# JOP-Lee/READ

Measured on AMD Instinct MI355X. Metric: rendered frames/sec @1216x352, 30M pts, higher is better.
Workload: dtype f32 (matrix-core products from two f16 pieces per operand, three piece pairs, fp32 accumulation)

## Files before the change

include/read_hip.h:

```cpp
#ifndef READ_HIP_H
#define READ_HIP_H

#include <stddef.h>
#include <stdint.h>

#ifdef __cplusplus
extern "C" {
#endif

#define READ_OK        0
#define READ_EINVAL  (-22)
#define READ_ENOMEM  (-12)
#define READ_EHIP     (-5)

#define READ_MAX_LEVELS      5
#define READ_DESC_CHANNELS   8

const char *read_last_error(void);
int read_abi_version(void);
int read_device_arch(char *name, int len);

int read_tuning_set(const char *key, int value);
int read_tuning_get(const char *key, int *value);
const char *read_tuning_key(int i);
// ... 190 lines not shown
    const float *wpacked_sc;
    int pre_bilinear;
    const void *wpacked_w4h;
    const void *wpacked_d3h;
    const void *wpacked_t3h;
} read_conv_desc;

size_t read_conv_packed_floats(int Cin, int Cout, int ksize);
size_t read_conv_param_floats(int Cout);
int read_conv_pack_weights_host(int Cin, int Cout, int ksize, int kc, const float *wf,
                                const float *wm, float *wpacked_host);
size_t read_conv_wino_floats(int Cin, int Cout);
int read_conv_pack_wino_host(int Cin, int Cout, const float *wf, const float *wm, float *wpacked_wino_host);
int read_conv_pack_w16_host(int Cin, int Cout, const float *wf, const float *wm, float *wpacked_w16_host);
size_t read_conv_w4_floats(int Cin, int Cout);
int read_conv_pack_w4_host(int Cin, int Cout, const float *wf, const float *wm, float *wpacked_w4_host);
size_t read_conv_w4h_floats(int Cin, int Cout);
int read_conv_pack_w4h_host(int Cin, int Cout, const float *wf, const float *wm, void *wpacked_w4h_host);
size_t read_conv_d3h_floats(int Cin, int Cout);
int read_conv_pack_d3h_host(int Cin, int Cout, const float *wf, const float *wm, void *wpacked_d3h_host);
size_t read_conv_dkh_floats(int Cin, int Cout, int ksize);
int read_conv_pack_dkh_host(int Cin, int Cout, int ksize, const float *wf, const float *wm, void *wpacked_host);
size_t read_conv_t3h_floats(int Cin, int Cout);
int read_conv_pack_t3h_host(int Cin, int Cout, const float *wf, const float *wm, void *wpacked_t3h_host);
size_t read_conv_sc_floats(int Cin, int Cout);
int read_conv_pack_sc_host(int Cin, int Cout, const float *wf, const float *wm, float *wpacked_sc_host);
int read_conv_pack_params_host(int Cout, const float *bf, const float *bm, const float *gamma,
                               const float *beta, const float *mean, const float *var, float eps,
                               float *params_host);
int read_gated_conv_forward(const read_conv_desc *desc, void *stream);
size_t read_conv_f4x1_floats(int Cin, int Cout);
int read_conv_pack_f4x1_host(int Cin, int Cout, const float *wf, const float *wm, void *wpacked_f4x1_host);
int read_gated_conv_forward_f4x1(const read_conv_desc *desc, const void *wpacked_f4x1, void *stream);
int read_conv_unpack_weights_host(int Cin, int Cout, int ksize, int kc, const float *wpacked_host, float *wf, float *wm);
int read_conv_kernel_family(const read_conv_desc *desc);
int read_conv_config_count(void);
const char *read_conv_config_name(int config);

int read_bilinear_up4(const float *in, int inH, int inW, int C, float *out, void *stream);

enum { READ_PACK_PARAMS = 0, READ_PACK_DIRECT = 1, READ_PACK_WINO = 2, READ_PACK_W4 = 3 };
typedef struct read_pack_job {
    int kind, mode;
    int Cin, Cout, ksize, kc;
    int Cp, first_block, nblocks;
    float eps;
    const float *wf, *wm;
    const float *bf, *bm, *gamma, *beta, *mean, *var;
    float *out;
    long long total;
} read_pack_job;
int read_conv_pack_job_prepare(read_pack_job *job);
int read_conv_pack_job(read_pack_job *job_host, void *stream);
int read_conv_pack_batch(const read_pack_job *jobs_dev, int njobs, int total_blocks, void *stream);
int read_conv_pack_params_device(int Cout, const float *bf, const float *bm, const float *gamma, const float *beta,
                                 const float *mean, const float *var, float eps, float *params, void *stream);
int read_conv_pack_weights_device(int Cin, int Cout, int ksize, int kc, const float *wf, const float *wm, float *wpacked,
                                  void *stream);
int read_conv_pack_wino_device(int Cin, int Cout, const float *wf, const float *wm, float *wpacked_wino, void *stream);
int read_conv_pack_w4_device(int Cin, int Cout, const float *wf, const float *wm, float *wpacked_w4, void *stream);
size_t read_conv_dgrad_packed_floats(int Cin, int Cout, int ksize);
size_t read_conv_dgrad_wino_floats(int Cin, int Cout);
size_t read_conv_dgrad_w4_floats(int Cin, int Cout);
int read_conv_pack_dgrad_device(int Cin, int Cout, int ksize, int kc, const float *wf, const float *wm, float *wpacked,
                                void *stream);
int read_conv_pack_dgrad_wino_device(int Cin, int Cout, const float *wf, const float *wm, float *wpacked_wino, void *stream);
// ... 68 lines not shown
```

read_amd/_lib.py:

```python
import ctypes as C
import os

_HERE = os.path.dirname(os.path.abspath(__file__))
LIB_PATH = os.path.join(_HERE, "libreadhip_debug.so" if os.environ.get("READ_HIP_DEBUG") else "libreadhip.so")
if os.environ.get("READ_HIP_VARIANT"):
    LIB_PATH = os.path.join(_HERE, "libreadhip_v_%s.so" % os.environ["READ_HIP_VARIANT"])

READ_MAX_LEVELS = 5
READ_CONV_MAX_SRC = 4
DESC_CHANNELS = 8


class ReadHipError(RuntimeError):
    pass


class ConvSrc(C.Structure):
    _fields_ = [("data", C.c_void_p), ("C", C.c_int), ("srcH", C.c_int), ("srcW", C.c_int), ("shift", C.c_int)]


class ConvDesc(C.Structure):
    _fields_ = [
        ("n_src", C.c_int), ("src", ConvSrc * READ_CONV_MAX_SRC), ("mul", C.c_void_p),
        ("inH", C.c_int), ("inW", C.c_int), ("Cout", C.c_int), ("ksize", C.c_int), ("stride", C.c_int),
# ... 117 lines not shown
    "read_rows_to_texture": (_i, [_vp, _i64, _i, _vp, _vp]),
    "read_gather_forward": (_i, [_vp, _i64, _i, _i, _pp, C.POINTER(_i64), _pp, _i, _vp]),
    "read_gather_forward_ss": (_i, [_vp, _i64, _i, _i, _i, _pp, C.POINTER(_i), C.POINTER(_i), _i, _pp, _i, _vp]),
    "read_gather_forward_tables": (_i, [C.POINTER(GatherTable), _i, _i, _i, _pp, C.POINTER(_i64), _pp, _vp]),
    "read_gather_backward": (_i, [_vp, _i64, _i, _i, _pp, C.POINTER(_i64), _pp, _vp]),
    "read_stitch_gather_forward": (_i, [C.POINTER(StitchPart), _i, _i, _i, C.POINTER(_i64), _pp, _pp, _pp, _pp, _vp]),
    "read_bilinear_down": (_i, [_vp, _i64, _i, _i, _i, _vp, _vp]),
    "read_bilinear_down_backward": (_i, [_vp, _i64, _i, _i, _i, _vp, _vp]),
    "read_conv_packed_floats": (_sz, [_i, _i, _i]),
    "read_conv_param_floats": (_sz, [_i]),
    "read_conv_pack_weights_host": (_i, [_i, _i, _i, _i, _vp, _vp, _vp]),
    "read_conv_pack_params_host": (_i, [_i, _vp, _vp, _vp, _vp, _vp, _vp, _f, _vp]),
    "read_conv_wino_floats": (_sz, [_i, _i]),
    "read_conv_pack_wino_host": (_i, [_i, _i, _vp, _vp, _vp]),
    "read_conv_pack_w16_host": (_i, [_i, _i, _vp, _vp, _vp]),
    "read_conv_w4_floats": (_sz, [_i, _i]),
    "read_conv_pack_w4_host": (_i, [_i, _i, _vp, _vp, _vp]),
    "read_conv_w4h_floats": (_sz, [_i, _i]),
    "read_conv_pack_w4h_host": (_i, [_i, _i, _vp, _vp, _vp]),
    "read_conv_d3h_floats": (_sz, [_i, _i]),
    "read_conv_pack_d3h_host": (_i, [_i, _i, _vp, _vp, _vp]),
    "read_conv_t3h_floats": (_sz, [_i, _i]),
    "read_conv_pack_t3h_host": (_i, [_i, _i, _vp, _vp, _vp]),
    "read_conv_dkh_floats": (_sz, [_i, _i, _i]),
    "read_conv_pack_dkh_host": (_i, [_i, _i, _i, _vp, _vp, _vp]),
    "read_gated_conv_forward": (_i, [C.POINTER(ConvDesc), _vp]),
    "read_conv_f4x1_floats": (_sz, [_i, _i]),
    "read_conv_unpack_weights_host": (_i, [_i, _i, _i, _i, _vp, _vp, _vp]),
    "read_unet_f4x1_floats": (_sz, []),
    "read_unet_f4x1_layer": (_i, [_i, C.POINTER(_sz), C.POINTER(_sz), C.POINTER(_i), C.POINTER(_i)]),
    "read_unet_set_f4x1": (_i, [_vp, _vp]),
    "read_conv_pack_f4x1_host": (_i, [_i, _i, _vp, _vp, _vp]),
    "read_gated_conv_forward_f4x1": (_i, [C.POINTER(ConvDesc), _vp, _vp]),
    "read_conv_kernel_family": (_i, [_vp]),
    "read_conv_sc_floats": (_sz, [_i, _i]),
    "read_conv_pack_sc_host": (_i, [_i, _i, _vp, _vp, _vp]),
    "read_conv_pack_job_prepare": (_i, [C.POINTER(PackJob)]),
    "read_conv_pack_job": (_i, [C.POINTER(PackJob), _vp]),
    "read_conv_pack_batch": (_i, [_vp, _i, _i, _vp]),
    "read_conv_config_count": (_i, []),
    "read_conv_config_name": (C.c_char_p, [_i]),
    "read_bilinear_up4": (_i, [_vp, _i, _i, _i, _vp, _vp]),
    "read_conv_pack_params_device": (_i, [_i, _vp, _vp, _vp, _vp, _vp, _vp, _f, _vp, _vp]),
    "read_conv_pack_weights_device": (_i, [_i, _i, _i, _i, _vp, _vp, _vp, _vp]),
    "read_conv_pack_wino_device": (_i, [_i, _i, _vp, _vp, _vp, _vp]),
    "read_conv_dgrad_wino_floats": (_sz, [_i, _i]),
    "read_conv_pack_dgrad_wino_device": (_i, [_i, _i, _vp, _vp, _vp, _vp]),
    "read_conv_pack_w4_device": (_i, [_i, _i, _vp, _vp, _vp, _vp]),
    "read_conv_dgrad_w4_floats": (_sz, [_i, _i]),
    "read_conv_pack_dgrad_w4_device": (_i, [_i, _i, _vp, _vp, _vp, _vp]),
    "read_conv_dgrad_packed_floats": (_sz, [_i, _i, _i]),
    "read_conv_pack_dgrad_device": (_i, [_i, _i, _i, _i, _vp, _vp, _vp, _vp]),
    "read_gate_forward": (_i, [_vp, _i64, _i, _vp, _i, _vp, _vp, _i, _i, _i, _vp]),
    "read_gate_backward": (_i, [_vp, _vp, _i64, _i, _vp, _i, _vp, _vp, _i, _i, _i, _vp]),
    "read_bn_param_grads": (_i, [_i, _vp, _vp, _vp, _f, _vp, _vp, _vp, _vp, _vp]),
    "read_bn_train_forward": (_i, [_vp, _i64, _i, _i, _i, _i, _i, _vp, _vp, _f, _f, _vp, _vp, _vp, _vp, _vp, _vp]),
    "read_gate_backward_bn": (_i, [_vp, _vp, _i64, _i, _vp, _i, _vp, _vp, _i, _i, _i, _i, _vp, _vp, _f, _vp, _vp]),
    "read_bn_param_grads_groups": (_i, [_i, _i, _vp, _vp, _f, _vp, _vp, _vp, _vp, _vp]),
    "read_conv_dgrad_generic_floats": (_sz, [_i, _i, _i]),
    "read_conv_dgrad_generic": (_i, [_vp, _i, _i, _i, _i, _i, _i, _vp, _vp, _vp, _i, _i, _vp, _vp]),
    "read_conv_wgrad_scratch_floats": (_sz, [_i, _i, _i, _i]),
    "read_conv_wgrad": (_i, [_vp, _i, _i, _i, _vp, _i, _i, _i, _vp, _vp, _i, _vp, _sz, _vp]),
    "read_conv_wgrad_family": (_i, [_i, _i, _i, _i, _i]),
    "read_bilinear_up4_blocks": (_i, [_vp, _i, _i, _i, _vp, _i, _i, _vp]),
    "read_bilinear_up4_backward": (_i, [_vp, _i, _i, _i, _vp, _i, _i, _vp]),
    "read_huber_loss": (_i, [_vp, _vp, _i64, _f, _vp, _vp, _vp]),
# ... 95 lines not shown
```

read_amd/csrc/conv.hip:

```cpp
#include <limits.h>

#include "common.h"
#include "internal.h"

using namespace readhip;

typedef float floatx16 __attribute__((ext_vector_type(16)));

namespace {

constexpr long long OOB_LIMIT = 0x7ffffff0ll;

struct SrcDev {
    const float *p;
    int C, H, W;
    int sl, sr;
};

struct ConvKArgs {
    SrcDev src[READ_CONV_MAX_SRC];
    const float *mul;
    const float *wp;
    const float *wp_wino;
    const float *wp_w16;
// ... 2179 lines not shown
                    const auto sw = __builtin_amdgcn_permlane32_swap(u0[k], u1[k], false, false);
                    u0[k] = sw[0];
                    u1[k] = sw[1];
                }
                Yf[py][px] = __builtin_bit_cast(f32x4, u0);
                Ym[py][px] = __builtin_bit_cast(f32x4, u1);
            }
#pragma unroll
        for (int py = 0; py < 2; ++py)
#pragma unroll
            for (int px = 0; px < 4; ++px) {
                f32x4 f = __builtin_elementwise_fma(Yf[py][px], isf, bf);
                const f32x4 mm = __builtin_elementwise_fma(Ym[py][px], ism, bml);
                if (a.elu) {
                    const f32x4 fe = f * LOG2E;
                    f32x4 e;
#pragma unroll
                    for (int k = 0; k < 4; ++k) e[k] = __builtin_amdgcn_exp2f(fe[k]);
                    e = e + f32x4{-1.0f, -1.0f, -1.0f, -1.0f};
#pragma unroll
                    for (int k = 0; k < 4; ++k) f[k] = f[k] > 0.0f ? f[k] : e[k];
                }
                f32x4 sg_, t;
#pragma unroll
                for (int k = 0; k < 4; ++k) t[k] = __builtin_amdgcn_exp2f(mm[k]);
                t = t + f32x4{1.0f, 1.0f, 1.0f, 1.0f};
#pragma unroll
                for (int k = 0; k < 4; ++k) sg_[k] = __builtin_amdgcn_rcpf(t[k]);
                const f32x4 v = (f * sg_) * sc + sh + rv[py][px];
                __builtin_amdgcn_raw_buffer_store_b128(__builtin_bit_cast(u32x4, v), out_rsrc, ovoff[py][px], 0, 0);
            }
        step_tile(by, bx);
        __builtin_amdgcn_s_setprio(0);
    }
}

struct D3hGeom {
    static constexpr int IH = 10, IW = 34, NPIX = IH * IW;
    static constexpr int XBUF = NPIX * 32;
    static constexpr int NE = NPIX * 8, NI = (NE + 511) / 512;
};

template <bool MUL>
__global__ __launch_bounds__(512, 1) void gated_conv_d3h_kernel(const ConvKArgs a)
{
    using DG = D3hGeom;
    __shared__ __attribute__((aligned(16))) unsigned lds[2 * DG::XBUF];
    __shared__ __attribute__((aligned(16))) float epar[6][32];
    const int tid = threadIdx.x, lane = tid & 63;
    const int wv = __builtin_amdgcn_readfirstlane(tid >> 6), rh = wv & 1, pq = wv >> 1;
    const SrcDev s = a.src[0];
    const int groups = a.CoutPad >> 5, G = gridDim.x;
    const int g = blockIdx.x % groups;
    const int n = a.nchunks;
    constexpr unsigned OOR = 0x80000000u;

    int by = (blockIdx.x / groups) / a.tiles_x, bx = (blockIdx.x / groups) % a.tiles_x;
    int pby = by, pbx = bx, pu = blockIdx.x, pchunk = 0;
    auto step_tile = [&](int &ty_, int &tx_) {
        ty_ += a.wino_dby;
        tx_ += a.wino_dbx;
        if (tx_ >= a.tiles_x) {
            tx_ -= a.tiles_x;
            ++ty_;
        }
    };
// ... 1119 lines not shown
    CFGW(1, 1, 32, 2, 1, 1, 2),
    CFGW(1, 1, 32, 1, 1, 1, 4),
    CFGW(3, 1, 8, 2, 1, 2, 2),
    {"k3s1c16_p1q1_wino", 3, 1, 16, 1, 1, 4, 1, 1, 2, gated_conv_wino_kernel<false, false>, gated_conv_wino_kernel<false, true>, 0, 0, 1},
    CFG(4, 2, 16, 1, 1, 1, 1, 1),
    CFG(4, 2, 16, 1, 1, 4, 1, 1),
    CFG(4, 2, 16, 1, 2, 2, 2, 1),
};
constexpr int N_CONFIGS = sizeof(g_configs) / sizeof(g_configs[0]);

int find_config(int ks, int s, int kc, int P, int QG, int WM, int WN, int PF, int NB)
{
    for (int i = 0; i < N_CONFIGS; ++i) {
        const ConvConfig &c = g_configs[i];
        if (c.KS == ks && c.S == s && c.KC == kc && c.P == P && c.QG == QG && c.WM == WM && c.WN == WN && c.PF == PF &&
            c.NB == NB)
            return i;
    }
    return -1;
}

enum ConvForce {
    CFG_AUTO = -1,
    CFG_PX = -2,
    CFG_W16 = -3,
    CFG_W4 = -5,
    CFG_SC = -6,
    CFG_W4H = -7,
    CFG_D3H = -8,
    CFG_D3H_S2 = -9,
    CFG_PXH = -10,
    CFG_T3H = -11,
    CFG_F4X1 = -12,
};

int g_prefer_wave = 1;
int g_wino_wgs = 2;
int g_conv_px = 1;
int g_kc32 = 1;
int g_use_wino = 1 << 30;
int g_w4_grid = 0;
int g_w4 = 32;
int g_w4h = 32;
int g_f4x1 = 32;
int g_d3h = 0;
int g_d3h_fam = 32;
int g_d3h_s2 = 32;
int g_pxh = 16;
int g_t3h = 8;
int g_sc = 8;
int g_w16 = 0;
int g_stagger_ticks = 0;

int find_wave_config(int ks, int s, int kc, int P, int QG)
{
    int best = -1;
    for (int i = 0; i < N_CONFIGS; ++i) {
        const ConvConfig &c = g_configs[i];
        if (c.wave && c.KS == ks && c.S == s && c.KC == kc && c.P == P && c.QG == QG) best = i;
    }
    return best;
}

int first_fit(int ks, int s, int kc, int groups, bool tiled_only = false, bool with_mul = false)
{
    for (int i = 0; i < N_CONFIGS; ++i) {
// ... 538 lines not shown
{
    g_trace = (unsigned long long *)buf;
    g_trace_records = buf ? bytes / 64 : 0;
}


static int conv_uses_wino(const read_conv_desc *d)
{
    return d->config < 0 && g_use_wino && !d->pre && d->ksize == 3 && d->stride == 1 && d->n_src == 1 &&
           d->src[0].shift == 0 && d->src[0].C % 16 == 0 && d->wpacked_wino && d->src[0].C <= g_use_wino;
}

static int conv_uses_w4(const read_conv_desc *d)
{
    const bool shape = !d->pre && (!d->linear || !d->residual) && d->ksize == 3 && d->stride == 1 && d->n_src == 1 && d->src[0].shift == 0 &&
                       d->src[0].C % 16 == 0 && d->src[0].C >= 32 && (d->Cout % 32 == 0 || (d->linear && d->Cout % 8 == 0)) && !d->fill_pad && d->wpacked_w4 &&
                       d->out_cstride % 4 == 0 &&
                       (long long)d->src[0].srcH * d->src[0].srcW * d->src[0].C * 4 < (1ll << 31) &&
                       (long long)d->inH * d->inW * d->out_cstride * 4 < (1ll << 31);
    return shape && (d->config == CFG_W4 || (d->config == CFG_AUTO && g_w4 > 0 && d->src[0].C >= g_w4));
}

static int conv_w4_shape(const read_conv_desc *d, const void *operand, bool with_threshold = false)
{
    read_conv_desc t = *d;
    if (!with_threshold) t.config = CFG_W4;
    t.wpacked_w4 = reinterpret_cast<const float *>(operand);
    return conv_uses_w4(&t);
}

static int conv_uses_w4h(const read_conv_desc *d)
{
    if (!d->wpacked_w4h || d->linear || d->mul || d->src[0].C % 32 != 0 || d->Cout % 32 != 0) return 0;
    const bool forced = d->config == CFG_W4H || d->config == CFG_F4X1;
    if (!forced && (d->config != CFG_AUTO || g_w4h <= 0 || d->src[0].C < g_w4h)) return 0;
    return conv_w4_shape(d, d->wpacked_w4h, !forced);
}

static int conv_uses_d3h(const read_conv_desc *d)
{
    if (!d->wpacked_d3h || d->linear || d->src[0].C % 32 != 0 || d->Cout % 32 != 0) return 0;
    const int min_c = d->mul ? g_d3h_fam : g_d3h;
    if (!(d->config == CFG_D3H || (d->config == CFG_AUTO && min_c > 0 && d->src[0].C >= min_c))) return 0;
    return conv_w4_shape(d, d->wpacked_d3h);
}

static int conv_uses_d3h_s2(const read_conv_desc *d)
{
    const bool shape = d->wpacked_d3h && !d->linear && !d->mul && !d->pre && !d->fill_pad && (d->ksize == 3 || d->ksize == 4) && d->stride == 2 && d->n_src == 1 &&
                       d->src[0].shift == 0 && d->src[0].C % 32 == 0 && d->Cout % 32 == 0 && d->out_cstride % 4 == 0 &&
                       (long long)d->src[0].srcH * d->src[0].srcW * d->src[0].C * 4 < (1ll << 31) &&
                       (long long)d->inH * d->inW * d->out_cstride * 4 < (1ll << 31);
    return shape && (d->config == CFG_D3H_S2 || (d->config == CFG_AUTO && g_d3h_s2 > 0 && d->src[0].C >= g_d3h_s2));
}

static int conv_uses_pxh(const read_conv_desc *d)
{
    if (!d->wpacked_d3h || d->ksize != 1 || d->stride != 1 || d->mul || d->fill_pad || d->n_src < 1 || d->n_src > READ_CONV_MAX_SRC) return 0;
    if (d->pre && d->pre_bilinear) return 0;
    int Cin = 0;
    for (int i = 0; i < d->n_src; ++i) {
        if (d->src[i].C < 8 || d->src[i].C % 8 != 0 || (uintptr_t)d->src[i].data % 16 != 0) return 0;
        Cin += d->src[i].C;
    }
    const bool shape = Cin % 16 == 0 && Cin <= 256 && d->Cout % 4 == 0 && d->out_cstride % 4 == 0 && (uintptr_t)d->out % 16 == 0 &&
                       (uintptr_t)d->params % 16 == 0 && (!d->residual || (uintptr_t)d->residual % 16 == 0) &&
                       (!d->pre || ((uintptr_t)d->pre % 16 == 0 && d->pre_cstride % 4 == 0 && d->pre_f_off % 4 == 0 && d->pre_m_off % 4 == 0));
// ... 36 lines not shown
    const bool fits = d->ksize == 1 && d->stride == 1 && !d->mul && !d->fill_pad && d->Cout % 4 == 0 && d->out_cstride % 4 == 0 &&
                      (uintptr_t)d->out % 16 == 0 && (uintptr_t)d->params % 16 == 0 && Cin / 8 <= 32 &&
                      (!d->residual || (uintptr_t)d->residual % 16 == 0) &&
                      (!d->pre || ((uintptr_t)d->pre % 16 == 0 && d->pre_cstride % 4 == 0 && d->pre_f_off % 4 == 0 && d->pre_m_off % 4 == 0));
    const bool bil = d->pre && d->pre_bilinear;
    return fits && (d->config == CFG_PX || (bil && d->config < 0) || (d->config == CFG_AUTO && g_conv_px && px_pick));
}

struct ConvShape {
    int Cin, kc;
    int outH, outW, CoutPad, groups;
};

static ConvShape conv_shape(const read_conv_desc *d)
{
    ConvShape s;
    s.Cin = 0;
    s.kc = 16;
    bool all32 = d->ksize == 1;
    for (int i = 0; i < d->n_src; ++i) {
        s.Cin += d->src[i].C;
        if (d->src[i].C % 16) s.kc = 8;
        all32 = all32 && d->src[i].C % 32 == 0;
    }
    if (all32 && (d->config >= 0 ? (d->config < N_CONFIGS && g_configs[d->config].KC == 32) : g_kc32 != 0)) s.kc = 32;
    const int pad = (d->ksize - 1) / 2;
    s.outH = (d->inH + 2 * pad - d->ksize) / d->stride + 1;
    s.outW = (d->inW + 2 * pad - d->ksize) / d->stride + 1;
    s.CoutPad = pad32(d->Cout);
    s.groups = s.CoutPad / 32;
    return s;
}

enum ConvKernel { CK_SC, CK_T3H, CK_PXH, CK_PX, CK_D3H_S2, CK_D3H, CK_F4X1, CK_W4H, CK_W4, CK_TABLE };

struct ConvRoute {
    ConvKernel kernel;
    int cfg;
    bool wino_auto;
    bool w16;
};

static ConvRoute conv_route(const read_conv_desc *d, const void *wp_f4x1)
{
    ConvRoute r = {CK_TABLE, -1, false, false};
    if (conv_uses_sc(d)) r.kernel = CK_SC;
    else if (conv_uses_t3h(d)) r.kernel = CK_T3H;
    else if (conv_uses_pxh(d)) r.kernel = CK_PXH;
    else if (conv_uses_px(d)) r.kernel = CK_PX;
    else if (conv_uses_d3h_s2(d)) r.kernel = CK_D3H_S2;
    else if (conv_uses_d3h(d)) r.kernel = CK_D3H;
    else if (conv_uses_w4h(d))
        r.kernel = wp_f4x1 && (d->config == CFG_F4X1 || (d->config == CFG_AUTO && g_f4x1 > 0 && d->src[0].C >= g_f4x1)) ? CK_F4X1 : CK_W4H;
    else if (conv_uses_w4(d)) r.kernel = CK_W4;
    else if (conv_sane(d)) {
        const ConvShape s = conv_shape(d);
        r.cfg = d->config;
        r.wino_auto = conv_uses_wino(d);
        for (int i = N_CONFIGS - 1; r.wino_auto && i >= 0; --i)
            if (g_configs[i].wino) r.cfg = i;
        if (d->linear && r.cfg < 0) r.cfg = first_fit(d->ksize, d->stride, s.kc, s.groups, true, d->mul != nullptr);
        if (r.cfg < 0) r.cfg = pick_config(d->ksize, d->stride, s.kc, s.groups, s.outH, s.outW);
        if (d->config < 0 && d->mul && r.cfg >= 0 && !g_configs[r.cfg].fn_mul) {
            const int m = first_fit(d->ksize, d->stride, s.kc, s.groups, false, true);
            if (m >= 0) r.cfg = m;
        }
        const bool mostly_padding = d->Cout <= 8;
        r.w16 = r.cfg >= 0 && r.cfg < N_CONFIGS && g_configs[r.cfg].wino && !d->linear && d->wpacked_w16 &&
                (d->config == CFG_W16 || (d->config < 0 && (g_w16 || mostly_padding)));
    }
    return r;
}

static int route_family(const ConvRoute &r)
{
    static const int family[] = { 1,  8,  7,  0,  6,  6,
                                  5,  5,  4,  0};
    return r.wino_auto ? 2 : family[r.kernel];
}

int conv_family(const read_conv_desc *d) { return route_family(conv_route(d, nullptr)); }

static int conv_prepare(const read_conv_desc *d, const void *wp_f4x1, ConvKArgs &a, ConvShape &s, ConvRoute &r)
{
    READ_CHECK_ARG(d, "read_gated_conv_forward: null descriptor");
    READ_CHECK_ARG(d->n_src >= 1 && d->n_src <= READ_CONV_MAX_SRC, "read_gated_conv_forward: n_src must be 1..%d",
                   READ_CONV_MAX_SRC);
    READ_CHECK_ARG(d->ksize == 1 || d->ksize == 3 || d->ksize == 4, "read_gated_conv_forward: ksize must be 1,3,4");
    READ_CHECK_ARG(d->stride == 1 || d->stride == 2, "read_gated_conv_forward: stride must be 1 or 2");
    READ_CHECK_ARG(d->inH >= 1 && d->inW >= 1 && d->Cout >= 1, "read_gated_conv_forward: bad sizes");
    READ_CHECK_ARG((d->wpacked || d->wpacked_w4 || d->wpacked_w4h || d->wpacked_d3h || d->wpacked_wino || d->wpacked_t3h || wp_f4x1) && d->params && d->out, "read_gated_conv_forward: null weights/params/out");
    READ_CHECK_ARG(d->out_cstride >= (d->linear ? 2 : 1) * d->Cout, "read_gated_conv_forward: out_cstride too small");
    READ_CHECK_ARG(!d->linear || (!d->residual && !d->fill_pad), "read_gated_conv_forward: linear mode takes no residual / fill");
    READ_CHECK_ARG(!d->mul || d->n_src == 1, "read_gated_conv_forward: mul needs a single source");
    READ_CHECK_ARG((uintptr_t)d->wpacked % 16 == 0, "read_gated_conv_forward: packed weights misaligned");
    r = conv_route(d, wp_f4x1);
    s = conv_shape(d);
    {
        const int family = route_family(r);
        const bool cfg_wino = d->config >= 0 && d->config < N_CONFIGS && g_configs[d->config].wino;
        const bool w16_forced = d->config == CFG_W16;
        READ_CHECK_ARG(d->wpacked || family != 0 || cfg_wino || w16_forced,
                       "read_gated_conv_forward: this launch takes a direct kernel and wpacked is NULL (fragment order not packed)");
        READ_CHECK_ARG(!d->wpacked || (!((const void *)d->wpacked == (const void *)d->wpacked_w4 && family != 4 && family != 5 && family != 6 && family != 7 && family != 8) &&
                                       !((const void *)d->wpacked == (const void *)d->wpacked_wino && family != 2 && !cfg_wino)),
                       "read_gated_conv_forward: wpacked aliases Winograd fragments but the launch takes kernel family %d "
                       "(ask read_conv_kernel_family before packing)", family);
        READ_CHECK_ARG(family != 4 || d->wpacked_w4, "read_gated_conv_forward: F(4x4) launch without wpacked_w4");
        READ_CHECK_ARG(family != 2 || d->wpacked_wino, "read_gated_conv_forward: F(2x2) launch without wpacked_wino");
        READ_CHECK_ARG(family != 1 || d->wpacked_sc, "read_gated_conv_forward: small-Cout launch without wpacked_sc");
// ... 133 lines not shown
    const int gw = (s.groups % 2 == 0 && nsteps <= 16) ? 2 : 1;
    const bool wide = g_conv_px == 2 || g_conv_px == 4;
    const int pt = (gw == 2 ? 1 : 2) * (wide ? 2 : 1);
    const size_t lds = (size_t)nsteps * 2 * gw * 1024;
    int per_cu = (int)((160 * 1024) / (lds + 256));
    const int reg_cap = wide ? 2 : 3;
    per_cu = per_cu < 1 ? 1 : per_cu > reg_cap ? reg_cap : per_cu;
    const int gsets = s.groups / gw;
    a.nchunks = nsteps;
    a.n_units = ceil_div(s.outH * s.outW, 32 * pt);
    const bool fullq = nsteps % 4 == 0;
    static const conv_fn fns[8] = {gated_conv_px_kernel<2, 1>, gated_conv_px_kernel<4, 1>, gated_conv_px_kernel<1, 2>, gated_conv_px_kernel<2, 2>,
                                   gated_conv_px_kernel<2, 1, true>, gated_conv_px_kernel<4, 1, true>, gated_conv_px_kernel<1, 2, true>, gated_conv_px_kernel<2, 2, true>};
    static bool attr_set[8] = {false, false, false, false, false, false, false, false};
    const int vi = (gw == 2 ? 2 : 0) + (wide ? 1 : 0) + (fullq ? 4 : 0);
    return launch_pixel_lane(fns[vi], attr_set[vi], 64 * 1024, n_cu * per_cu, gsets, false, lds, stream, a);
}

static int take_out_gated(const read_conv_desc *d, bool winograd, ConvKArgs &a)
{
    READ_CHECK_ARG(!d->out_gated || (winograd && d->linear && (uintptr_t)d->out_gated % 16 == 0 && d->block_h >= 0 &&
                                     d->valid_h <= d->block_h),
                   "read_gated_conv_forward: out_gated needs a linear launch on the Winograd kernel");
    a.out_gated = d->out_gated;
    a.blk_h = d->block_h;
    a.blk_valid = d->valid_h;
    return READ_OK;
}

static int refuse_f4x1_config(const read_conv_desc *d, bool f4x1)
{
    READ_CHECK_ARG(d->config != CFG_F4X1 || f4x1, "read_gated_conv_forward: config -12 takes the launches of the split-operand 3x3/s1 family "
                   "and needs the F(4,3)-by-rows operand (read_gated_conv_forward_f4x1)");
    return READ_OK;
}

static int persistent_grid(ConvKArgs &a, int groups, int cap)
{
    int nwg = a.n_units < cap ? a.n_units : cap;
    nwg -= nwg % groups;
    if (nwg < groups) nwg = groups;
    a.wino_dby = (nwg / groups) / a.tiles_x;
    a.wino_dbx = (nwg / groups) % a.tiles_x;
    return nwg;
}

static int launch_d3h_s2(const read_conv_desc *d, ConvKArgs &a, const ConvShape &s, hipStream_t stream)
{
    const int rc = take_out_gated(d, false, a);
    if (rc != READ_OK) return rc;
    READ_CHECK_ARG((uintptr_t)d->wpacked_d3h % 16 == 0, "read_gated_conv_forward: wpacked_d3h misaligned");
    a.wp_d3h = d->wpacked_d3h;
    a.nchunks = s.Cin / 32;
    a.tiles_x = ceil_div(s.outW, 16);
    const int pairs = (s.CoutPad + 63) / 64;
    a.n_units = a.tiles_x * ceil_div(s.outH, 8) * pairs;
    const int nwg = persistent_grid(a, pairs, device_cus());
    if (d->ksize == 4) hipLaunchKernelGGL((gated_conv_d3h_s2_kernel<4>), dim3((unsigned)nwg), dim3(512), 0, stream, a);
    else hipLaunchKernelGGL((gated_conv_d3h_s2_kernel<3>), dim3((unsigned)nwg), dim3(512), 0, stream, a);
    READ_CHECK_LAUNCH();
    return READ_OK;
}

static int launch_w4_family(const read_conv_desc *d, ConvKArgs &a, const ConvShape &s, ConvKernel kernel, const void *wp_f4x1, hipStream_t stream)
{
    const bool d3h = kernel == CK_D3H, f4x1 = kernel == CK_F4X1, w4h = f4x1 || kernel == CK_W4H;
    int rc = take_out_gated(d, kernel == CK_W4, a);
    if (rc != READ_OK) return rc;
    rc = refuse_f4x1_config(d, f4x1);
    if (rc != READ_OK) return rc;
    READ_CHECK_ARG(!w4h || f4x1 || d->wpacked_w4h != wp_f4x1, "read_gated_conv_forward: this launch takes the F(4x4) split-operand kernel "
                   "and only the F(4,3)-by-rows order was packed");
    READ_CHECK_ARG((uintptr_t)(d3h ? d->wpacked_d3h : w4h ? d->wpacked_w4h : (const void *)d->wpacked_w4) % 16 == 0,
                   "read_gated_conv_forward: wpacked_w4 / wpacked_w4h / wpacked_d3h misaligned");
    a.wp_d3h = d->wpacked_d3h;
    READ_CHECK_ARG(!d->mul || (uintptr_t)d->mul % 16 == 0, "read_gated_conv_forward: mul misaligned");
    a.wp_w4h = d->wpacked_w4h;
    a.wp_f4x1 = wp_f4x1;
    READ_CHECK_ARG(!f4x1 || (uintptr_t)wp_f4x1 % 16 == 0, "read_gated_conv_forward: wpacked_f4x1 misaligned");
    a.nchunks = (w4h || d3h) ? s.Cin / 32 : s.Cin / s.kc;
    a.tiles_x = ceil_div(s.outW, 32);
    a.n_units = a.tiles_x * ceil_div(s.outH, 8) * s.groups;
    const int n_cu = device_cus(), groups = s.groups;
    int cap = n_cu;
    if (g_w4_grid) {
        const int whole = n_cu - n_cu % groups > 0 ? n_cu - n_cu % groups : groups;
        cap = ceil_div(ceil_div(a.n_units, ceil_div(a.n_units, whole)), groups) * groups;
        if (cap > n_cu) cap -= groups;
    }
    const int nwg = persistent_grid(a, groups, cap);
    conv_fn fn = d->linear ? (d->out_gated ? gated_conv_wino4_kernel<false, 1> : gated_conv_wino4_kernel<false, 2>) : d->mul ? gated_conv_wino4_kernel<true> : gated_conv_wino4_kernel<false>;
    unsigned threads = 256;
    if (d3h) {
        fn = d->mul ? gated_conv_d3h_kernel<true> : gated_conv_d3h_kernel<false>;
        threads = 512;
    } else if (f4x1) fn = gated_conv_f4x1h_kernel;
    else if (w4h) fn = gated_conv_wino4h_kernel;
    READ_CHECK_ARG(!d->linear || !d->mul, "read_gated_conv_forward: linear launches take no multiplier");
    hipLaunchKernelGGL(fn, dim3((unsigned)nwg), dim3(threads), 0, stream, a);
    READ_CHECK_LAUNCH();
    return READ_OK;
}

static int launch_table(const read_conv_desc *d, ConvKArgs &a, const ConvShape &s, const ConvRoute &r, hipStream_t stream)
{
    const int groups = s.groups;
    READ_CHECK_ARG(!d->linear || d->config < 0 || (d->config < N_CONFIGS && !g_configs[d->config].wave),
                   "read_gated_conv_forward: linear mode needs a workgroup-tiled or Winograd config");
    READ_CHECK_ARG(r.cfg >= 0 && r.cfg < N_CONFIGS, "read_gated_conv_forward: no kernel for k=%d s=%d kc=%d groups=%d",
                   d->ksize, d->stride, s.kc, groups);
    const ConvConfig &c = g_configs[r.cfg];
    READ_CHECK_ARG(c.KS == d->ksize && c.S == d->stride && c.KC == s.kc && groups % (c.WN * c.QG) == 0,
                   "read_gated_conv_forward: config %s does not fit k=%d s=%d kc=%d groups=%d", c.name, d->ksize,
                   d->stride, s.kc, groups);
    a.nchunks = s.Cin / s.kc;
    a.tiles_x = ceil_div(s.outW, 32);
    READ_CHECK_ARG(!d->pre || !c.wino, "read_gated_conv_forward: the Winograd kernel takes no pre-activation addend");
    int rc = take_out_gated(d, c.wino != 0, a);
    if (rc != READ_OK) return rc;
    const int tiles_y = ceil_div(s.outH, c.WM * c.P);
    dim3 grid((unsigned)(a.tiles_x * tiles_y), (unsigned)(groups / (c.WN * c.QG)));
    a.trace = ((size_t)grid.x * grid.y <= g_trace_records) ? g_trace : nullptr;
    if (c.wino) {
        READ_CHECK_ARG(d->wpacked_wino && (uintptr_t)d->wpacked_wino % 16 == 0, "read_gated_conv_forward: config %s needs wpacked_wino", c.name);
        READ_CHECK_ARG(d->n_src == 1 && d->src[0].shift == 0 && d->src[0].C % 16 == 0,
                       "read_gated_conv_forward: the Winograd kernel takes one un-resampled source with C %% 16 == 0");
        a.tiles_x = ceil_div(s.outW, 16);
        a.n_units = a.tiles_x * ceil_div(s.outH, 8) * groups;
        grid = dim3((unsigned)persistent_grid(a, groups, g_wino_wgs * device_cus()), 1);
        a.trace = ((size_t)grid.x * 4 <= g_trace_records) ? g_trace : nullptr;
    }
    if (c.wave) {
        a.tiles_y = ceil_div(s.outH, c.P);
        a.trace = nullptr;
        a.stagger_ticks = g_stagger_ticks;
        a.col_split = a.tiles_x * (groups / c.QG);
        a.n_full = a.col_split * a.tiles_y;
        a.n_units = a.n_full;
        const int want = ceil_div(a.n_units, 4), cap = device_cus() * c.wg_per_cu;
        grid = dim3((unsigned)(want < cap ? want : cap), 1);
    }
    rc = refuse_f4x1_config(d, false);
    if (rc != READ_OK) return rc;
    conv_fn fn = c.fn;
    if (c.wino && a.trace && !d->mul) fn = gated_conv_wino_kernel<true, false>;
    if (d->mul) {
        READ_CHECK_ARG(c.fn_mul, "read_gated_conv_forward: config %s has no multiply variant", c.name);
        READ_CHECK_ARG((uintptr_t)d->mul % 16 == 0, "read_gated_conv_forward: mul misaligned");
        fn = c.fn_mul;
    }
    if (r.w16 && !a.trace) {
        READ_CHECK_ARG((uintptr_t)d->wpacked_w16 % 16 == 0, "read_gated_conv_forward: wpacked_w16 misaligned");
        fn = d->mul ? gated_conv_wino16s_kernel<true> : gated_conv_wino16s_kernel<false>;
    }
    hipLaunchKernelGGL(fn, grid, dim3(256), 0, stream, a);
    READ_CHECK_LAUNCH();
    return READ_OK;
}

int launch_gated_conv(const read_conv_desc *d, hipStream_t stream, const void *wp_f4x1)
{
    ConvKArgs a;
    ConvShape s;
    ConvRoute r;
    const int rc = conv_prepare(d, wp_f4x1, a, s, r);
    if (rc != READ_OK) return rc;
    switch (r.kernel) {
    case CK_SC: return launch_sc(d, a, s, stream);
    case CK_T3H:
    case CK_PXH: return launch_pxh(d, a, s, r.kernel == CK_T3H, stream);
    case CK_PX: return launch_px(a, s, stream);
    case CK_D3H_S2: return launch_d3h_s2(d, a, s, stream);
    case CK_D3H:
    case CK_F4X1:
    case CK_W4H:
    case CK_W4: return launch_w4_family(d, a, s, r.kernel, wp_f4x1, stream);
    case CK_TABLE: return launch_table(d, a, s, r, stream);
    }
    return READ_EINVAL;
}

}

extern "C" int read_conv_kernel_family(const read_conv_desc *desc) { return desc ? readhip::conv_family(desc) : -1; }

extern "C" int read_gated_conv_forward_f4x1(const read_conv_desc *desc, const void *wpacked_f4x1, void *stream)
{
    if (!desc || !wpacked_f4x1 || desc->wpacked_w4h) return readhip::launch_gated_conv(desc, as_stream(stream), wpacked_f4x1);
    read_conv_desc t = *desc;
    t.wpacked_w4h = wpacked_f4x1;
    return readhip::launch_gated_conv(&t, as_stream(stream), wpacked_f4x1);
}

extern "C" int read_gated_conv_forward(const read_conv_desc *desc, void *stream)
{
    return readhip::launch_gated_conv(desc, as_stream(stream), nullptr);
}

namespace {
__global__ __launch_bounds__(256, 1) void mfma_f32_rate_kernel(float *out, int iters)
{
    f32x4 acc[16];
#pragma unroll
    for (int i = 0; i < 16; ++i) acc[i] = f32x4{0.f, 0.f, 0.f, 0.f};
    float a0 = 0.37f + 0.001f * threadIdx.x, b0 = 1.0f - 0.002f * threadIdx.x;
    for (int it = 0; it < iters; ++it) {
#pragma unroll
        for (int m = 0; m < 16; ++m) acc[m] = __builtin_amdgcn_mfma_f32_16x16x4f32(a0, b0, acc[m], 0, 0, 0);
        a0 = a0 * 0.999f + 0.0007f;
        b0 = b0 * 1.0001f - 0.0001f;
    }
    float s = 0.f;
#pragma unroll
    for (int i = 0; i < 16; ++i) s += acc[i][0] + acc[i][3];
    if (s == 1234.5678f) out[blockIdx.x * 256 + threadIdx.x] = s;
// ... 30 lines not shown
```

Measured before the change: 309.7.

## Add two-workgroups-per-CU F(4,3) split-operand conv kernel with auto routing

Adds a new persistent F(4,3)-by-rows Winograd gated conv kernel with launch bounds allowing two workgroups per CU. It holds fewer weight and B-operand registers in flight and uses a smaller ring, so that two workgroups can overlap their latencies. The launch grid is doubled to twice the CU count. Auto routing picks it when there are more tiles than CUs and Cin is 32 or 128. Cutting per-block register buffering to fit two blocks may add stalls inside each block, and the routing heuristic is narrow.

New measurement: 317.6, median of 6. 2.5% higher.

```diff
diff --git a/include/read_hip.h b/include/read_hip.h
--- a/include/read_hip.h
+++ b/include/read_hip.h
@@ -246,6 +246,7 @@
 size_t read_conv_f4x1_floats(int Cin, int Cout);
 int read_conv_pack_f4x1_host(int Cin, int Cout, const float *wf, const float *wm, void *wpacked_f4x1_host);
 int read_gated_conv_forward_f4x1(const read_conv_desc *desc, const void *wpacked_f4x1, void *stream);
+int read_conv_f4x1_pair_occupancy(void);
 int read_conv_unpack_weights_host(int Cin, int Cout, int ksize, int kc, const float *wpacked_host, float *wf, float *wm);
 int read_conv_kernel_family(const read_conv_desc *desc);
 int read_conv_config_count(void);
diff --git a/read_amd/_lib.py b/read_amd/_lib.py
--- a/read_amd/_lib.py
+++ b/read_amd/_lib.py
@@ -173,6 +173,7 @@
     "read_unet_set_f4x1": (_i, [_vp, _vp]),
     "read_conv_pack_f4x1_host": (_i, [_i, _i, _vp, _vp, _vp]),
     "read_gated_conv_forward_f4x1": (_i, [C.POINTER(ConvDesc), _vp, _vp]),
+    "read_conv_f4x1_pair_occupancy": (_i, []),
     "read_conv_kernel_family": (_i, [_vp]),
     "read_conv_sc_floats": (_sz, [_i, _i]),
     "read_conv_pack_sc_host": (_i, [_i, _i, _vp, _vp, _vp]),
diff --git a/read_amd/csrc/conv.hip b/read_amd/csrc/conv.hip
--- a/read_amd/csrc/conv.hip
+++ b/read_amd/csrc/conv.hip
@@ -2235,6 +2235,269 @@
             }
         step_tile(by, bx);
         __builtin_amdgcn_s_setprio(0);
+    }
+}
+
+__global__ __launch_bounds__(256, 2) void f4x1_pair_conv_kernel(const ConvKArgs a)
+{
+    using WG = F4x1Geom;
+    __shared__ __attribute__((aligned(16))) unsigned lds[WG::VBUF];
+    __shared__ __attribute__((aligned(16))) float epar[6][32];
+    const int tid = threadIdx.x, lane = tid & 63;
+    const int wv = __builtin_amdgcn_readfirstlane(tid >> 6);
+    const SrcDev s = a.src[0];
+    const int groups = a.CoutPad >> 5, G = gridDim.x;
+    const int g = blockIdx.x % groups;
+    const int n = a.nchunks;
+
+    int by = (blockIdx.x / groups) / a.tiles_x, bx = (blockIdx.x / groups) % a.tiles_x;
+    int pby = by, pbx = bx, pu = blockIdx.x, pchunk = 0;
+    auto step_tile = [&](int &ty_, int &tx_) {
+        ty_ += a.wino_dby;
+        tx_ += a.wino_dbx;
+        if (tx_ >= a.tiles_x) {
+            tx_ -= a.tiles_x;
+            ++ty_;
+        }
+    };
+
+    const int cp = lane & 15, sg = (wv & 1) * 4 + (lane >> 4);
+    constexpr unsigned OOR = 0x80000000u;
+    unsigned xoff[6];
+    int rowoff[5];
+    bool rowok[5];
+    const unsigned src_bytes = (unsigned)(a.inH * s.W * s.C) * 4u;
+    const auto rsrc = __builtin_amdgcn_make_buffer_rsrc(const_cast<float *>(s.p), 0, src_bytes, 0x00020000);
+    auto set_patch = [&]() {
+        const int y0 = pby * 8 - 1 + (wv >> 1), x0 = pbx * 32 + 4 * sg - 1;
+#pragma unroll
+        for (int i = 0; i < 5; ++i) {
+            const int yy = y0 + 2 * i;
+            rowok[i] = (unsigned)yy < (unsigned)a.inH;
+            const int yc = yy < 0 ? 0 : yy >= a.inH ? a.inH - 1 : yy;
+            rowoff[i] = yc * s.W * s.C * 4;
+        }
+#pragma unroll
+        for (int c = 0; c < 6; ++c) xoff[c] = (unsigned)(x0 + c) < (unsigned)a.inW ? (unsigned)((x0 + c) * s.C + 2 * cp) * 4u : OOR;
+    };
+    auto advance = [&]() {
+        if (++pchunk == n) {
+            pchunk = 0;
+            if (pu + G < a.n_units) {
+                pu += G;
+                step_tile(pby, pbx);
+            }
+            set_patch();
+        }
+    };
+    f32x2 d2[5][6];
+    const auto rsrc_none = __builtin_amdgcn_make_buffer_rsrc(const_cast<float *>(s.p), 0, 0, 0x00020000);
+    auto gload_patch = [&]() {
+#pragma unroll
+        for (int i = 0; i < 5; ++i)
+#pragma unroll
+            for (int c = 0; c < 6; ++c)
+                d2[i][c] = __builtin_bit_cast(f32x2, __builtin_amdgcn_raw_buffer_load_b64(rowok[i] ? rsrc : rsrc_none, xoff[c], rowoff[i] + pchunk * 128, 0));
+    };
+    auto bt6 = [](f32x2 &x0, f32x2 &x1, f32x2 &x2, f32x2 &x3, f32x2 &x4, f32x2 &x5) {
+        const f32x2 p = pk_add(x3, x4), q = pk_add(x1, x2), r = pk_sub(x4, x3), u = pk_sub(x1, x2), f = pk_sub(x3, x1), h = pk_sub(x4, x2);
+        const f32x2 y0 = __builtin_elementwise_fma(x2, f32x2{-5.0f, -5.0f}, __builtin_elementwise_fma(x0, f32x2{4.0f, 4.0f}, x4));
+        const f32x2 y5 = __builtin_elementwise_fma(x3, f32x2{-5.0f, -5.0f}, __builtin_elementwise_fma(x1, f32x2{4.0f, 4.0f}, x5));
+        x0 = y0;
+        x1 = __builtin_elementwise_fma(q, f32x2{-4.0f, -4.0f}, p);
+        x2 = __builtin_elementwise_fma(u, f32x2{4.0f, 4.0f}, r);
+        x3 = __builtin_elementwise_fma(f, f32x2{2.0f, 2.0f}, h);
+        x4 = __builtin_elementwise_fma(f, f32x2{-2.0f, -2.0f}, h);
+        x5 = y5;
+    };
+    const int vwoff = (wv >> 1) * WG::VROW + sg * 16 + (((cp >> 2) ^ ((-wv) & 3)) << 2) + (cp & 3);
+    auto split_store = [&](const f32x2 x, int i, int fq) {
+        unsigned hi, lo;
+        float r0, r1;
+        asm("v_cvt_pk_f16_f32 %0, %1, %2" : "=v"(hi) : "v"(x.x), "v"(x.y));
+        asm("v_fma_mix_f32 %0, %1, -1.0, %2 op_sel_hi:[1,0,0]" : "=v"(r0) : "v"(hi), "v"(x.x));
+        asm("v_fma_mix_f32 %0, %1, -1.0, %2 op_sel:[1,0,0] op_sel_hi:[1,0,0]" : "=v"(r1) : "v"(hi), "v"(x.y));
+        const f32x2 rs = f32x2{r0, r1} * f32x2{2048.0f, 2048.0f};
+        asm("v_cvt_pk_f16_f32 %0, %1, %2" : "=v"(lo) : "v"(rs.x), "v"(rs.y));
+        lds[vwoff + 2 * i * WG::VROW + fq * WG::VFREQ] = hi;
+        lds[vwoff + 2 * i * WG::VROW + fq * WG::VFREQ + 128] = lo;
+    };
+
+    const char *const wbase = reinterpret_cast<const char *>(a.wp_f4x1) + ((size_t)(g * 4 + wv) * n) * (18 * 2048);
+    const auto wrsrc = __builtin_amdgcn_make_buffer_rsrc(const_cast<char *>(wbase), 0, (unsigned)n * (18 * 2048), 0x00020000);
+    const unsigned wvoff = lane * 16;
+    constexpr int RW = 6;
+    u32x4 Wh[RW], Wl[RW];
+    f16x8 Ws;
+    auto wload = [&](int chunk, int fq, int ky) {
+        const int slot = (fq & 1) * 3 + ky;
+        Wh[slot] = __builtin_amdgcn_raw_buffer_load_b128(wrsrc, wvoff, ((chunk * 3 + ky) * 6 + fq) * 2048, 0);
+        Wl[slot] = __builtin_amdgcn_raw_buffer_load_b128(wrsrc, wvoff, ((chunk * 3 + ky) * 6 + fq) * 2048 + 1024, 0);
+    };
+    auto wscale = [&](int fq, int ky) {
+        const _Float16 k = (_Float16)0x1p-11f;
+        Ws = __builtin_bit_cast(f16x8, Wh[(fq & 1) * 3 + ky]) * f16x8{k, k, k, k, k, k, k, k};
+    };
+    const int t16 = lane & 15, kl = lane >> 4;
+    const int vrd_e = (t16 >> 3) * WG::VROW + (t16 & 7) * 16 + ((kl ^ ((-(t16 >> 2)) & 3)) << 2);
+    const int vrd_o = (t16 >> 3) * WG::VROW + (t16 & 7) * 16 + ((kl ^ ((-((t16 >> 2) ^ 2)) & 3)) << 2);
+    constexpr int RB = 3;
+    u32x4 Bh[RB], Bl[RB];
+    auto bload = [&](int idx) {
+        const int fq = idx / 9, sp = idx % 9;
+        const int o = sp * WG::VROW + fq * WG::VFREQ + ((sp & 1) ? vrd_o : vrd_e);
+        Bh[idx % RB] = *reinterpret_cast<const u32x4 *>(__builtin_assume_aligned(lds + o, 16));
+        Bl[idx % RB] = *reinterpret_cast<const u32x4 *>(__builtin_assume_aligned(lds + o + 128, 16));
+    };
+
+    f32x4 acc[4][6];
+    const auto out_rsrc = __builtin_amdgcn_make_buffer_rsrc(a.out, 0, (unsigned)(a.outH * a.outW * a.out_cstride) * 4u, 0x00020000);
+    const auto res_rsrc = __builtin_amdgcn_make_buffer_rsrc(const_cast<float *>(a.residual ? a.residual : a.out), 0,
+                                                            (unsigned)(a.outH * a.outW * a.Cout) * 4u, 0x00020000);
+    const float *const wsc = reinterpret_cast<const float *>(a.wp_f4x1) + (size_t)n * 1152 * a.CoutPad;
+    if (tid < 192) {
+        constexpr float L2E = 1.44269504088896341f;
+        const int arr = tid >> 5, c = g * 32 + (tid & 31);
+        const float v = arr < 4 ? a.params[arr * a.CoutPad + c] : wsc[(arr - 4) * a.CoutPad + c];
+        epar[arr][tid & 31] = (arr == 1 || arr == 5) ? v * -L2E : v;
+    }
+
+    set_patch();
+    gload_patch();
+
+    auto stage_body = [&](int chunk) {
+        __syncthreads();
+#pragma unroll
+        for (int ky = 0; ky < 3; ++ky) wload(chunk, 0, ky);
+#pragma unroll
+        for (int i = 0; i < 5; ++i) {
+            bt6(d2[i][0], d2[i][1], d2[i][2], d2[i][3], d2[i][4], d2[i][5]);
+#pragma unroll
+            for (int fq = 0; fq < 6; ++fq) split_store(d2[i][fq], i, fq);
+        }
+        __syncthreads();
+        bload(0);
+        bload(1);
+        wscale(0, 0);
+        __builtin_amdgcn_sched_barrier(0);
+#pragma unroll
+        for (int fq = 0; fq < 6; ++fq)
+#pragma unroll
+            for (int sp = 0; sp < 9; ++sp)
+#pragma unroll
+                for (int q = 0; q < 2; ++q) {
+                    const int nb = (sp & 1) ? sp >> 1 : (sp >> 1) - 1 + q, ky = (sp & 1) ? 1 : q ? 0 : 2;
+                    if (((sp & 1) && q) || nb < 0 || nb > 3) continue;
+#pragma unroll
+                    for (int pc = 0; pc < 3; ++pc) {
+                        const int mb = 3 * sp + 3 * ((sp > 0 ? sp - 1 : 0) / 2);
+                        const int ms = mb + ((!(sp & 1) && q && sp > 0) ? 3 : 0) + pc, idx = fq * 9 + sp;
+                        if (ms == mb && idx + 2 < 54) bload(idx + 2);
+                        const int ws = (fq & 1) * 3 + ky;
+                        const f16x8 av = pc == 0 ? Ws : __builtin_bit_cast(f16x8, pc == 1 ? Wl[ws] : Wh[ws]);
+                        const f16x8 bv = __builtin_bit_cast(f16x8, pc == 0 ? Bl[idx % RB] : Bh[idx % RB]);
+                        acc[nb][fq] = __builtin_amdgcn_mfma_f32_16x16x32_f16(av, bv, acc[nb][fq], 0, 0, 0);
+                        if (fq < 5 && (ms == 5 || ms == 11 || ms == 17)) wload(chunk, fq + 1, (ms - 5) / 6);
+                        if (pc == 1) {
+                            if (ms < 33) wscale(fq, (ms / 3 + 1) % 3);
+                            else if (fq < 5) wscale(fq + 1, 0);
+                        }
+                        __builtin_amdgcn_sched_barrier(0);
+                    }
+                }
+    };
+
+    for (int u = blockIdx.x; u < a.n_units; u += G) {
+#pragma unroll
+        for (int nb = 0; nb < 4; ++nb)
+#pragma unroll
+            for (int fq = 0; fq < 6; ++fq) asm volatile("v_accvgpr_write_b32 %0, 0\n\tv_accvgpr_write_b32 %1, 0\n\tv_accvgpr_write_b32 %2, 0\n\tv_accvgpr_write_b32 %3, 0"
+                                                        : "=a"(acc[nb][fq][0]), "=a"(acc[nb][fq][1]), "=a"(acc[nb][fq][2]), "=a"(acc[nb][fq][3]));
+        for (int chunk = 0; chunk < n; ++chunk) {
+            stage_body(chunk);
+            if (chunk + 1 < n) {
+                advance();
+                gload_patch();
+            }
+        }
+
+        int ln;
+        asm volatile("v_mbcnt_lo_u32_b32 %0, -1, 0\n\tv_mbcnt_hi_u32_b32 %0, -1, %0" : "=v"(ln));
+        const int e16 = ln & 15, cq = (ln >> 4) & 1, hf = ln >> 5;
+        const int c0 = g * 32 + wv * 8 + 4 * cq;
+        const int oy = by * 8 + 4 * hf + (e16 >> 3), ox = bx * 32 + 4 * (e16 & 7);
+        const int cl = wv * 8 + 4 * cq;
+        const f32x4 bf = *reinterpret_cast<const f32x4 *>(&epar[0][cl]), bml = *reinterpret_cast<const f32x4 *>(&epar[1][cl]);
+        const f32x4 sc = *reinterpret_cast<const f32x4 *>(&epar[2][cl]), sh = *reinterpret_cast<const f32x4 *>(&epar[3][cl]);
+        const f32x4 isf = *reinterpret_cast<const f32x4 *>(&epar[4][cl]), ism = *reinterpret_cast<const f32x4 *>(&epar[5][cl]);
+        constexpr float LOG2E = 1.44269504088896341f;
+        asm volatile("s_nop 15\n\ts_nop 3");
+#pragma unroll
+        for (int py = 0; py < 2; ++py) {
+            unsigned rvoff[4], ovoff[4];
+#pragma unroll
+            for (int px = 0; px < 4; ++px) {
+                const bool in = (oy + 2 * py < a.outH) & (ox + px < a.outW) & (c0 < a.Cout);
+                const int pix = (oy + 2 * py) * a.outW + ox + px;
+                rvoff[px] = in ? (unsigned)((pix * a.Cout + c0) * 4) : OOR;
+                ovoff[px] = in ? (unsigned)((pix * a.out_cstride + c0) * 4) : OOR;
+            }
+            f32x4 rv[4];
+#pragma unroll
+            for (int px = 0; px < 4; ++px) {
+                rv[px] = f32x4{0.f, 0.f, 0.f, 0.f};
+                if (a.residual) rv[px] = __builtin_bit_cast(f32x4, __builtin_amdgcn_raw_buffer_load_b128(res_rsrc, rvoff[px], 0, 0));
+            }
+            f32x4 Y[2][4];
+#pragma unroll
+            for (int h = 0; h < 2; ++h) {
+                f32x4 m[6];
+#pragma unroll
+                for (int fq = 0; fq < 6; ++fq)
+#pragma unroll
+                    for (int k = 0; k < 4; ++k) asm volatile("v_accvgpr_read_b32 %0, %1" : "=v"(m[fq][k]) : "a"(acc[py + 2 * h][fq][k]));
+                const f32x4 s1 = m[1] + m[2], d1 = pk_sub4(m[1], m[2]);
+                const f32x4 s2 = m[3] + m[4], dd2 = pk_sub4(m[3], m[4]);
+                Y[h][0] = m[0] + s1 + s2;
+                Y[h][1] = d1 + 2.0f * dd2;
+                Y[h][2] = s1 + 4.0f * s2;
+                Y[h][3] = d1 + 8.0f * dd2 + m[5];
+                __builtin_amdgcn_sched_barrier(0);
+            }
+#pragma unroll
+            for (int px = 0; px < 4; ++px) {
+                u32x4 u0 = __builtin_bit_cast(u32x4, Y[0][px]), u1 = __builtin_bit_cast(u32x4, Y[1][px]);
+#pragma unroll
+                for (int k = 0; k < 4; ++k) {
+                    const auto sw = __builtin_amdgcn_permlane32_swap(u0[k], u1[k], false, false);
+                    u0[k] = sw[0];
+                    u1[k] = sw[1];
+                }
+                f32x4 f = __builtin_elementwise_fma(__builtin_bit_cast(f32x4, u0), isf, bf);
+                const f32x4 mm = __builtin_elementwise_fma(__builtin_bit_cast(f32x4, u1), ism, bml);
+                if (a.elu) {
+                    const f32x4 fe = f * LOG2E;
+                    f32x4 e;
+#pragma unroll
+                    for (int k = 0; k < 4; ++k) e[k] = __builtin_amdgcn_exp2f(fe[k]);
+                    e = e + f32x4{-1.0f, -1.0f, -1.0f, -1.0f};
+#pragma unroll
+                    for (int k = 0; k < 4; ++k) f[k] = f[k] > 0.0f ? f[k] : e[k];
+                }
+                f32x4 sg_, t;
+#pragma unroll
+                for (int k = 0; k < 4; ++k) t[k] = __builtin_amdgcn_exp2f(mm[k]);
+                t = t + f32x4{1.0f, 1.0f, 1.0f, 1.0f};
+#pragma unroll
+                for (int k = 0; k < 4; ++k) sg_[k] = __builtin_amdgcn_rcpf(t[k]);
+                const f32x4 v = (f * sg_) * sc + sh + rv[px];
+                __builtin_amdgcn_raw_buffer_store_b128(__builtin_bit_cast(u32x4, v), out_rsrc, ovoff[px], 0, 0);
+                __builtin_amdgcn_sched_barrier(0);
+            }
+        }
+        step_tile(by, bx);
+        advance();
+        gload_patch();
     }
 }
 
@@ -3420,6 +3683,7 @@
     CFG_PXH = -10,
     CFG_T3H = -11,
     CFG_F4X1 = -12,
+    CFG_F4X1_PAIR = -13,
 };
 
 int g_prefer_wave = 1;
@@ -4024,7 +4288,7 @@
 static int conv_uses_w4h(const read_conv_desc *d)
 {
     if (!d->wpacked_w4h || d->linear || d->mul || d->src[0].C % 32 != 0 || d->Cout % 32 != 0) return 0;
-    const bool forced = d->config == CFG_W4H || d->config == CFG_F4X1;
+    const bool forced = d->config == CFG_W4H || d->config == CFG_F4X1 || d->config == CFG_F4X1_PAIR;
     if (!forced && (d->config != CFG_AUTO || g_w4h <= 0 || d->src[0].C < g_w4h)) return 0;
     return conv_w4_shape(d, d->wpacked_w4h, !forced);
 }
@@ -4127,7 +4391,7 @@
     return s;
 }
 
-enum ConvKernel { CK_SC, CK_T3H, CK_PXH, CK_PX, CK_D3H_S2, CK_D3H, CK_F4X1, CK_W4H, CK_W4, CK_TABLE };
+enum ConvKernel { CK_SC, CK_T3H, CK_PXH, CK_PX, CK_D3H_S2, CK_D3H, CK_F4X1, CK_F4X1_PAIR, CK_W4H, CK_W4, CK_TABLE };
 
 struct ConvRoute {
     ConvKernel kernel;
@@ -4135,6 +4399,10 @@
     bool wino_auto;
     bool w16;
 };
+
+static int w4_units(const ConvShape &s) { return ceil_div(s.outW, 32) * ceil_div(s.outH, 8) * s.groups; }
+
+static bool f4x1_pair_auto(int Cin, int n_units, int n_cu) { return n_units > n_cu && (Cin == 32 || Cin == 128); }
 
 static ConvRoute conv_route(const read_conv_desc *d, const void *wp_f4x1)
 {
@@ -4145,8 +4413,13 @@
     else if (conv_uses_px(d)) r.kernel = CK_PX;
     else if (conv_uses_d3h_s2(d)) r.kernel = CK_D3H_S2;
     else if (conv_uses_d3h(d)) r.kernel = CK_D3H;
-    else if (conv_uses_w4h(d))
-        r.kernel = wp_f4x1 && (d->config == CFG_F4X1 || (d->config == CFG_AUTO && g_f4x1 > 0 && d->src[0].C >= g_f4x1)) ? CK_F4X1 : CK_W4H;
+    else if (conv_uses_w4h(d)) {
+        const bool forced = d->config == CFG_F4X1 || d->config == CFG_F4X1_PAIR;
+        const bool f4x1 = wp_f4x1 && (forced || (d->config == CFG_AUTO && g_f4x1 > 0 && d->src[0].C >= g_f4x1));
+        const bool pair = f4x1 && (d->config == CFG_F4X1_PAIR ||
+                                   (d->config == CFG_AUTO && f4x1_pair_auto(d->src[0].C, w4_units(conv_shape(d)), device_cus())));
+        r.kernel = !f4x1 ? CK_W4H : pair ? CK_F4X1_PAIR : CK_F4X1;
+    }
     else if (conv_uses_w4(d)) r.kernel = CK_W4;
     else if (conv_sane(d)) {
         const ConvShape s = conv_shape(d);
@@ -4170,7 +4443,7 @@
 static int route_family(const ConvRoute &r)
 {
     static const int family[] = { 1,  8,  7,  0,  6,  6,
-                                  5,  5,  4,  0};
+                                  5,  5,  5,  4,  0};
     return r.wino_auto ? 2 : family[r.kernel];
 }
 
@@ -4370,6 +4643,8 @@
 {
     READ_CHECK_ARG(d->config != CFG_F4X1 || f4x1, "read_gated_conv_forward: config -12 takes the launches of the split-operand 3x3/s1 family "
                    "and needs the F(4,3)-by-rows operand (read_gated_conv_forward_f4x1)");
+    READ_CHECK_ARG(d->config != CFG_F4X1_PAIR || f4x1, "read_gated_conv_forward: config -13 takes the launches of the split-operand 3x3/s1 family "
+                   "and needs the F(4,3)-by-rows operand (read_gated_conv_forward_f4x1)");
     return READ_OK;
 }
 
@@ -4402,7 +4677,7 @@
 
 static int launch_w4_family(const read_conv_desc *d, ConvKArgs &a, const ConvShape &s, ConvKernel kernel, const void *wp_f4x1, hipStream_t stream)
 {
-    const bool d3h = kernel == CK_D3H, f4x1 = kernel == CK_F4X1, w4h = f4x1 || kernel == CK_W4H;
+    const bool d3h = kernel == CK_D3H, pair = kernel == CK_F4X1_PAIR, f4x1 = pair || kernel == CK_F4X1, w4h = f4x1 || kernel == CK_W4H;
     int rc = take_out_gated(d, kernel == CK_W4, a);
     if (rc != READ_OK) return rc;
     rc = refuse_f4x1_config(d, f4x1);
@@ -4418,8 +4693,8 @@
     READ_CHECK_ARG(!f4x1 || (uintptr_t)wp_f4x1 % 16 == 0, "read_gated_conv_forward: wpacked_f4x1 misaligned");
     a.nchunks = (w4h || d3h) ? s.Cin / 32 : s.Cin / s.kc;
     a.tiles_x = ceil_div(s.outW, 32);
-    a.n_units = a.tiles_x * ceil_div(s.outH, 8) * s.groups;
-    const int n_cu = device_cus(), groups = s.groups;
+    a.n_units = w4_units(s);
+    const int n_cu = (pair ? 2 : 1) * device_cus(), groups = s.groups;
     int cap = n_cu;
     if (g_w4_grid) {
         const int whole = n_cu - n_cu % groups > 0 ? n_cu - n_cu % groups : groups;
@@ -4432,7 +4707,8 @@
     if (d3h) {
         fn = d->mul ? gated_conv_d3h_kernel<true> : gated_conv_d3h_kernel<false>;
         threads = 512;
-    } else if (f4x1) fn = gated_conv_f4x1h_kernel;
+    } else if (pair) fn = f4x1_pair_conv_kernel;
+    else if (f4x1) fn = gated_conv_f4x1h_kernel;
     else if (w4h) fn = gated_conv_wino4h_kernel;
     READ_CHECK_ARG(!d->linear || !d->mul, "read_gated_conv_forward: linear launches take no multiplier");
     hipLaunchKernelGGL(fn, dim3((unsigned)nwg), dim3(threads), 0, stream, a);
@@ -4496,6 +4772,12 @@
     return READ_OK;
 }
 
+int f4x1_pair_occupancy()
+{
+    int n = 0;
+    return hipOccupancyMaxActiveBlocksPerMultiprocessor(&n, f4x1_pair_conv_kernel, 256, 0) == hipSuccess ? n : -1;
+}
+
 int launch_gated_conv(const read_conv_desc *d, hipStream_t stream, const void *wp_f4x1)
 {
     ConvKArgs a;
@@ -4511,6 +4793,7 @@
     case CK_D3H_S2: return launch_d3h_s2(d, a, s, stream);
     case CK_D3H:
     case CK_F4X1:
+    case CK_F4X1_PAIR:
     case CK_W4H:
     case CK_W4: return launch_w4_family(d, a, s, r.kernel, wp_f4x1, stream);
     case CK_TABLE: return launch_table(d, a, s, r, stream);
@@ -4519,6 +4802,8 @@
 }
 
 }
+
+extern "C" int read_conv_f4x1_pair_occupancy(void) { return readhip::f4x1_pair_occupancy(); }
 
 extern "C" int read_conv_kernel_family(const read_conv_desc *desc) { return desc ? readhip::conv_family(desc) : -1; }
 
```
